# kopacja/rho2sdf.jl

Measured on AMD Instinct MI355X. Metric: Mvoxels/s SDF extract on 512^3 grid over 100k HEX8; max|err| vs ref, higher is better.
Workload: dtype f64

## Files before the change

rho2sdf.jl_amd/csrc/rho2sdf_hip.hip:

```cpp
#include <hip/hip_runtime.h>

#include <algorithm>
#include <cmath>
#include <cstdarg>
#include <cstddef>
#include <cstdio>
#include <cstring>
#include <initializer_list>
#include <utility>
#include <string>
#include <vector>

#include "../../include/rho2sdf_hip.h"
#include "r2s_common.hpp"
#include "r2s_device_math.hpp"

#include <type_traits>

using namespace r2s;

__constant__ int c_hex_isn[6][4] = {{0, 3, 2, 1}, {0, 1, 5, 4}, {1, 2, 6, 5},
                                    {2, 3, 7, 6}, {3, 0, 4, 7}, {4, 5, 6, 7}};

#define SCAN_BLOCK 256
// ... 1305 lines not shown
            for (int k = 0; k < 8; ++k) t = fma(E.X[k][q], N[k], t);
            xp[q] = t;
        }
        res[slot] = norm3(x[0] - xp[0], x[1] - xp[1], x[2] - xp[2]);
        if (res_xp) {
            res_xp[3 * slot] = xp[0];
            res_xp[3 * slot + 1] = xp[1];
            res_xp[3 * slot + 2] = xp[2];
        }
    }
}

struct alignas(16) SignBox {
    int32_t lo[3];
    int32_t dim[3];
    double rmax;
};

__device__ __forceinline__ bool coord_range(const GridDev& g, int ax, double mn, double mx, int nmax, int& a, int& b)
{
    const double fa = ceil((mn - g.amin[ax]) / g.cell), fb = floor((mx - g.amin[ax]) / g.cell);
    if (!(fa <= (double)nmax + 2.0) || !(fb >= -2.0)) return false;
    a = (fa < 0.0) ? 0 : ((fa > (double)nmax) ? nmax : (int)fa);
    b = (fb > (double)nmax) ? nmax : ((fb < 0.0) ? 0 : (int)fb);
    while (a > 0 && grid_coord(g, ax, a - 1) >= mn) --a;
    while (a <= nmax && grid_coord(g, ax, a) < mn) ++a;
    while (b < nmax && grid_coord(g, ax, b + 1) <= mx) ++b;
    while (b >= 0 && grid_coord(g, ax, b) > mx) --b;
    return a <= b;
}

__global__ void sign_box_kernel(const ElemRec* __restrict__ erec, uint32_t nel, GridDev g, SlabInfo s,
                                const uint8_t* __restrict__ hot, SignBox* __restrict__ sbox,
                                uint32_t* __restrict__ nchunks, uint32_t* __restrict__ nstore)
{
    const uint32_t gid = blockIdx.x * blockDim.x + threadIdx.x;
    const uint32_t el = gid / BIN_LANES, sub = gid % BIN_LANES;
    const bool live = el < nel;
    SignBox B;
    memset(&B, 0, sizeof B);
    const ElemRec& E = erec[live ? el : 0];
    int lo[3], hi[3];
    bool found = false;
    if (live && sign_tile_range(E, g, s, lo, hi)) {
        const uint32_t n = tile_count(lo, hi);
        for (uint32_t q = sub; q < n && !found; q += BIN_LANES) found = hot[tile_of(lo, hi, q, s)] != 0;
    }
    const unsigned long long m = __ballot(found);
    const bool rel = ((m >> ((threadIdx.x & 63u) & ~(unsigned)(BIN_LANES - 1))) & ((1ull << BIN_LANES) - 1ull)) != 0;
    if (!live || sub != 0) return;
    if (rel) {
        const int nmax[3] = {g.nx - 1, g.ny - 1, g.nz - 1};
        uint64_t vol = 1;
        for (int ax = 0; ax < 3; ++ax) {
            int a = 0, b = -1;
            if (coord_range(g, ax, E.mn[ax], E.mx[ax], nmax[ax], a, b)) {
                if (ax == 2) {
                    int la, lb;
                    if (slab_local_range(s, a, b, la, lb)) { a = la; b = lb; }
                    else { a = 0; b = -1; }
                }
            } else { a = 0; b = -1; }
            B.lo[ax] = a;
            B.dim[ax] = (b >= a) ? (b - a + 1) : 0;
            vol *= (uint64_t)B.dim[ax];
        }
        if (vol == 0) B.dim[0] = B.dim[1] = B.dim[2] = 0;
        nchunks[el] = (uint32_t)((vol + 63) / 64);
        const TileBox tb = tile_box(B.lo, B.dim);
        nstore[el] = vol ? (uint32_t)(tb.td[0] * tb.td[1] * tb.td[2]) : 0u;
    }
    B.rmax = E.rmax;
    sbox[el] = B;
}

__global__ void __launch_bounds__(64) sign_project_kernel(const SignBox* __restrict__ sbox, uint32_t nel,
                                                          const uint32_t* __restrict__ chunk_off, uint32_t nchunks,
                                                          const uint32_t* __restrict__ store_off,
                                                          uint32_t cpw, const ElemRec* __restrict__ erec, GridDev g,
                                                          SlabInfo sl, double rho_t, const uint8_t* __restrict__ hot,
                                                          double* __restrict__ res, const uint32_t* __restrict__ abort_flag)
{
    const uint32_t ab = *abort_flag;
    __shared__ uint32_t queue[128];
    const uint32_t w = __builtin_amdgcn_readfirstlane((blockIdx.x * blockDim.x + threadIdx.x) >> 6);
    uint32_t c = w * cpw;
    if (c >= nchunks) return;
    const uint32_t c_end = (c + cpw < nchunks) ? c + cpw : nchunks;
    uint32_t lo = 0, hi = nel;
    while (hi - lo > 1) {
        const uint32_t mid = (lo + hi) >> 1;
        if (chunk_off[mid] <= c) lo = mid; else hi = mid;
    }
    if (ab) return;
    const uint32_t lane = threadIdx.x & 63;
    while (c < c_end) {
        lo = __builtin_amdgcn_readfirstlane(lo);
        const SignBox& B = sbox[lo];
        const ElemRec& E = erec[lo];
        const uint32_t co = chunk_off[lo], cn = chunk_off[lo + 1];
        const uint32_t seg_end = (cn < c_end) ? cn : c_end;
        const BoxDecode dec = box_decode_make((uint32_t)B.dim[0], (uint32_t)B.dim[1], (uint32_t)B.dim[2]);
        const uint32_t vol = dec.bxy * (uint32_t)B.dim[2];
        const uint32_t v_begin = (c - co) * 64u;
        const uint32_t v_end = ((seg_end - co) * 64u < vol) ? (seg_end - co) * 64u : vol;
        const int lo0 = B.lo[0], lo1 = B.lo[1], lo2 = B.lo[2];
        const uint32_t st_off = store_off[lo];
        const TileBox tb = tile_box(B.lo, B.dim);
        const double margin = 1e-9 * fmax(1.0, fabs(rho_t));
        const double uniform_sign = (E.rmin > rho_t + margin) ? 1.0 : ((E.rmax < rho_t - margin) ? -1.0 : 0.0);
        uint32_t qn = 0;
        for (uint32_t v0 = v_begin; v0 < v_end || qn > 0; v0 += 64u) {
            if (v0 < v_end) {
                const uint32_t v = v0 + lane;
                bool pass = false;
                if (v < v_end) {
                    uint32_t li, lj, lk;
                    box_decode(dec, v, li, lj, lk);
                    const int i = lo0 + (int)li, j = lo1 + (int)lj, kl = lo2 + (int)lk;
                    double x[3];
                    x[0] = grid_coord(g, 0, i);
                    x[1] = grid_coord(g, 1, j);
                    x[2] = grid_coord(g, 2, slab_global_k(sl, kl));
                    const uint32_t t = ((uint32_t)(kl >> 2) * sl.nty + (uint32_t)(j >> 2)) * sl.ntx + (uint32_t)(i >> 2);
                    pass = hot[t] && !hex8_outside(E, x);
                    if (!pass) res[tile_slot(st_off, tb, i, j, kl)] = INFINITY;
                    else if (uniform_sign != 0.0 && hex8_inner(E, x)) {
                        res[tile_slot(st_off, tb, i, j, kl)] = uniform_sign > 0.0 ? 0.0 : -0.0;
                        pass = false;
                    }
                }
                const uint64_t m = __ballot(pass);
                if (pass) queue[qn + __builtin_amdgcn_mbcnt_hi((uint32_t)(m >> 32), __builtin_amdgcn_mbcnt_lo((uint32_t)m, 0u))] = v;
                qn += (uint32_t)__popcll(m);
                __syncthreads();
            }
            if (qn >= 64u || (v0 + 64u >= v_end && qn > 0)) {
                const uint32_t take = qn < 64u ? qn : 64u;
                const bool have = lane < take;
                const uint32_t v = queue[lane];
                const uint32_t spill = queue[64u + lane];
                __syncthreads();
                if (lane + 64u < qn) queue[lane] = spill;
                qn -= take;
                __syncthreads();
                if (have) {
                    uint32_t li, lj, lk;
                    box_decode(dec, v, li, lj, lk);
                    const int i = lo0 + (int)li, j = lo1 + (int)lj, kl = lo2 + (int)lk;
                    double x[3], xi[3], N[8];
                    x[0] = grid_coord(g, 0, i);
                    x[1] = grid_coord(g, 1, j);
                    x[2] = grid_coord(g, 2, slab_global_k(sl, kl));
                    inv_map_hex8(E, x, xi);
                    const double m = fmax(fabs(xi[0]), fmax(fabs(xi[1]), fabs(xi[2])));
                    double val = INFINITY;
                    if (m < 1.01) {
                        hex8_shape(xi, N);
                        double rho = 0.0;
#pragma unroll
                        for (int k = 0; k < 8; ++k) rho += N[k] * E.r[k];
                        val = (rho >= rho_t) ? m : -m;
                    }
                    res[tile_slot(st_off, tb, i, j, kl)] = val;
                }
            }
        }
        c = seg_end;
        if (c < c_end) {
            do { ++lo; } while (chunk_off[lo + 1] <= c);
        }
    }
}

#define AT_ITEMS 8
__global__ void __launch_bounds__(256) active_tiles_kernel(const uint32_t* __restrict__ band_cnt,
                                                           const uint32_t* __restrict__ sign_cnt,
                                                           const uint8_t* __restrict__ hot, uint32_t ntiles,
                                                           uint32_t* __restrict__ active_band,
                                                           uint32_t* __restrict__ active_sign,
                                                           uint32_t* __restrict__ active_any,
                                                           uint32_t* __restrict__ active_sonly,
                                                           const uint8_t* __restrict__ tri,
                                                           uint32_t* __restrict__ active_lean,
                                                           uint32_t* __restrict__ active_tri,
                                                           uint32_t* __restrict__ counters)
{
    __shared__ uint32_t s_cnt[6][AT_ITEMS][4], s_base[6], s_max[2];
    if (threadIdx.x < 2) s_max[threadIdx.x] = 0;
    const int lane = threadIdx.x & 63, wave = threadIdx.x >> 6;
    const unsigned long long below = (1ull << lane) - 1ull;
    const uint32_t t0 = blockIdx.x * (256u * AT_ITEMS);
    uint32_t mxb = 0, mxs = 0;
    uint32_t flags[AT_ITEMS];
#pragma unroll
    for (int i = 0; i < AT_ITEMS; ++i) {
        const uint32_t t = t0 + (uint32_t)i * 256u + threadIdx.x;
        const bool in = t < ntiles;
        const uint32_t bc = in ? band_cnt[t] : 0u, sc = in ? sign_cnt[t] : 0u;
        const bool f[3] = {bc != 0, sc != 0 && hot[t] != 0, false};
        const bool ft = f[0] && tri[t] != 0;
        const bool fl[6] = {f[0], f[1], f[0] || f[1], f[1] && !f[0], f[0] && !ft, ft};
        uint32_t fb = 0;
// ... 388 lines not shown
    const uint32_t* __restrict__ ids = reinterpret_cast<const uint32_t*>(seg + 2 + (int64_t)cap_full * 64);
    const int lane = threadIdx.x & 63;
    const int ntx = (nx + 3) / 4, nty = (ny + 3) / 4;
    const uint32_t t = ids[w];
    const int tx = t % ntx, ty = (t / ntx) % nty, tz = t / (ntx * nty);
    const int i = tx * 4 + (lane & 3), j = ty * 4 + ((lane >> 2) & 3), k = tz * 4 + (lane >> 4);
    if (i < nx && j < ny && k < nz) volume[((int64_t)k * ny + j) * nx + i] = payload[(size_t)w * 64 + lane];
}
__global__ void __launch_bounds__(256) unpack_segments_masks_kernel(const double* __restrict__ buf, int64_t seglen, uint32_t cap_full,
                                                                   uint32_t cap_mask, int nx, int ny, int nz, double magnitude,
                                                                   double* __restrict__ volume)
{
    const double* __restrict__ seg = buf + (int64_t)blockIdx.y * seglen;
    const int64_t nf = reinterpret_cast<const int64_t*>(seg)[0], nm = reinterpret_cast<const int64_t*>(seg)[1];
    const uint32_t w = __builtin_amdgcn_readfirstlane((blockIdx.x * blockDim.x + threadIdx.x) >> 6);
    if (nf < 0 || nf > (int64_t)cap_full || nm < 0 || nm > (int64_t)cap_mask || (int64_t)w >= nm) return;
    const uint64_t* __restrict__ masks = reinterpret_cast<const uint64_t*>(seg + 2 + (int64_t)cap_full * 64 + (cap_full + 1) / 2);
    const uint32_t* __restrict__ ids = reinterpret_cast<const uint32_t*>(masks + cap_mask);
    const int lane = threadIdx.x & 63;
    const int ntx = (nx + 3) / 4, nty = (ny + 3) / 4;
    const uint32_t t = ids[w];
    const int tx = t % ntx, ty = (t / ntx) % nty, tz = t / (ntx * nty);
    const int i = tx * 4 + (lane & 3), j = ty * 4 + ((lane >> 2) & 3), k = tz * 4 + (lane >> 4);
    if (i < nx && j < ny && k < nz) volume[((int64_t)k * ny + j) * nx + i] = ((masks[w] >> lane) & 1ull) ? magnitude : -magnitude;
}

struct r2s_plan {
    int device = 0;
    int n_cu = 256;
    DevBuf deg, ine_ptr, ine, cursor, erec, cls, fmask, nitems, item_off, items;
    DevBuf band_cnt, band_off, band_raw, band_ent, sign_cnt, sign_off, sign_raw, sign_ent;
    DevBuf active, active_sign, active_any, active_sonly, active_lean, active_tri, tri, hot, counters, scan_tmp[3], scan_tmp2[3], nchunks, chunk_off, iso_res, iso_res_xp, strag;
    DevBuf perm, wchunks, hardflag;
    DevBuf sbox, s_nchunks, s_chunk_off, sres;
    DevBuf nstore, store_off, s_nstore, s_store_off;
    SlabInfo last_s;
    GridDev last_g;
    uint32_t last_n_any = 0, last_n_band = 0, last_n_sonly = 0;
    bool has_last = false;
    uint32_t* h_pinned = nullptr;
    uint32_t* d_pinned = nullptr;
    struct Spec {
        bool valid = false;
        int64_t key[12] = {0};
        uint32_t v[16] = {0};
    } spec;
    hipEvent_t ev[8] = {nullptr, nullptr, nullptr, nullptr, nullptr, nullptr, nullptr, nullptr};
    hipStream_t st2 = nullptr;
    hipStream_t st3 = nullptr;
    hipEvent_t ev2[8] = {nullptr, nullptr, nullptr, nullptr, nullptr, nullptr, nullptr, nullptr};
    hipEvent_t ev_fast[2] = {nullptr, nullptr};
    bool fast_timed = false;
};

static int scan_exclusive2(r2s_plan* P, const uint32_t* in0, uint32_t* out0, const uint32_t* in1, uint32_t* out1,
                           int64_t n, hipStream_t st, int level = 0, int bank = 0)
{
    DevBuf* tmp = bank ? P->scan_tmp2 : P->scan_tmp;
    if (n <= 0) return 0;
    const unsigned ny = in1 ? 2u : 1u;
    const int64_t nb = (n + SCAN_TILE - 1) / SCAN_TILE;
    ScanPair sp;
    sp.in[0] = in0; sp.out[0] = out0; sp.in[1] = in1; sp.out[1] = out1;
    sp.sums[0] = sp.sums[1] = nullptr;
    if (nb == 1) {
        scan_block_kernel<<<dim3(1, ny), SCAN_BLOCK, 0, st>>>(sp, n);
        return 0;
// ... 108 lines not shown
    int rc = check_device(device);
    if (rc) return rc;
    HIP_TRY(hipSetDevice(device));
    r2s_plan* P = new r2s_plan();
    P->device = device;
    {
        hipDeviceProp_t prop;
        if (hipGetDeviceProperties(&prop, device) == hipSuccess && prop.multiProcessorCount > 0) P->n_cu = prop.multiProcessorCount;
    }
    HIP_TRY(hipHostMalloc((void**)&P->h_pinned, 128, hipHostMallocMapped | hipHostMallocCoherent));
    HIP_TRY(hipHostGetDevicePointer((void**)&P->d_pinned, P->h_pinned, 0));
    for (int i = 0; i < 8; ++i) HIP_TRY(hipEventCreate(&P->ev[i]));
    for (int i = 0; i < 8; ++i) HIP_TRY(hipEventCreate(&P->ev2[i]));
    for (int i = 0; i < 2; ++i) HIP_TRY(hipEventCreate(&P->ev_fast[i]));
    {
        int prio_lo = 0, prio_hi = 0;
        HIP_TRY(hipDeviceGetStreamPriorityRange(&prio_lo, &prio_hi));
        (void)prio_lo;
        HIP_TRY(hipStreamCreateWithPriority(&P->st2, hipStreamNonBlocking, prio_hi));
        HIP_TRY(hipStreamCreateWithFlags(&P->st3, hipStreamNonBlocking));
    }
    *out = P;
    return 0;
}

void r2s_plan_destroy(r2s_plan* P)
{
    if (!P) return;
    (void)hipSetDevice(P->device);
    DevBuf* all[] = {&P->deg, &P->ine_ptr, &P->ine, &P->cursor, &P->erec, &P->cls, &P->fmask, &P->nitems,
                     &P->item_off, &P->items, &P->band_cnt, &P->band_off, &P->band_raw, &P->band_ent,
                     &P->sign_cnt, &P->sign_off, &P->sign_raw, &P->sign_ent, &P->active, &P->active_sign, &P->active_any, &P->active_sonly, &P->active_lean, &P->active_tri, &P->tri,
                     &P->hot, &P->counters, &P->nchunks, &P->chunk_off, &P->iso_res, &P->iso_res_xp, &P->strag,
                     &P->perm, &P->wchunks, &P->hardflag, &P->sbox, &P->s_nchunks, &P->s_chunk_off, &P->sres, &P->nstore, &P->store_off, &P->s_nstore, &P->s_store_off,
                     &P->scan_tmp[0], &P->scan_tmp[1], &P->scan_tmp[2], &P->scan_tmp2[0], &P->scan_tmp2[1], &P->scan_tmp2[2]};
    for (DevBuf* b : all) b->release();
    if (P->h_pinned) (void)hipHostFree(P->h_pinned);
    for (int i = 0; i < 8; ++i)
        if (P->ev[i]) (void)hipEventDestroy(P->ev[i]);
    for (int i = 0; i < 8; ++i)
        if (P->ev2[i]) (void)hipEventDestroy(P->ev2[i]);
    for (int i = 0; i < 2; ++i)
        if (P->ev_fast[i]) (void)hipEventDestroy(P->ev_fast[i]);
    if (P->st2) (void)hipStreamDestroy(P->st2);
    if (P->st3) (void)hipStreamDestroy(P->st3);
    delete P;
}


}

static uint32_t iso_straggler_cap(uint32_t n_store)
{
    static const int cap_env = getenv("R2S_ISO_STRAGGLER_CAP") ? atoi(getenv("R2S_ISO_STRAGGLER_CAP")) : 0;
    if (cap_env > 0) return (uint32_t)cap_env;
    const uint64_t slots = 64ull * std::max<uint32_t>(n_store, 1u);
    return (uint32_t)std::max<uint64_t>(slots / 16, std::min<uint64_t>(slots, 1ull << 20));
}

static int iso_project_hex(r2s_plan* P, hipStream_t st, uint32_t n_items, uint32_t n_chunks, uint32_t n_store, uint32_t wps,
                           const GridDev& g, const SlabInfo& s, double rho_t, double* res_xp, uint32_t* counters,
                           const uint32_t* abort_flag)
{
    static const int free_env = getenv("R2S_ISO_FREE") ? atoi(getenv("R2S_ISO_FREE")) : 0;
    const uint32_t resident = (uint32_t)P->n_cu * 4u * wps - (uint32_t)std::min(std::max(free_env, 0), (int)P->n_cu * 4);
    static const int group_env = getenv("R2S_ISO_GROUP") ? atoi(getenv("R2S_ISO_GROUP")) : 0;
    const uint32_t group = group_env > 0 ? (uint32_t)group_env
// ... 125 lines not shown
    elem_prep_kernel<ET><<<(unsigned)((nel + 127) / 128), 128, 0, st>>>(
        dX, dIEN, d_rho_n, nel, nnp, rho_t, g, P->erec.as<typename ET::Rec>(),
        P->cls.as<uint8_t>(), P->fmask.as<uint32_t>(), P->nitems.as<uint32_t>(), s, delta);
    HIP_TRY(hipEventRecord(P->ev2[5], st));
    HIP_TRY(hipStreamWaitEvent(P->st2, P->ev2[0], 0));
    {
        const int64_t n = nel * ET::NEN;
        node_degree_kernel<<<(unsigned)((n + 255) / 256), 256, 0, P->st2>>>(dIEN, nel, ET::NEN, nnp, P->deg.as<uint32_t>(), (int*)counters);
        int rc = scan_exclusive(P, P->deg.as<uint32_t>(), P->ine_ptr.as<uint32_t>(), nnp + 1, P->st2);
        if (rc) return rc;
        ine_fill_kernel<<<(unsigned)((n + 255) / 256), 256, 0, P->st2>>>(dIEN, nel, ET::NEN, nnp, P->ine_ptr.as<uint32_t>(), P->cursor.as<uint32_t>(), P->ine.as<uint32_t>());
    }
    HIP_TRY(hipEventRecord(P->ev2[1], P->st2));
    if constexpr (std::is_same<typename ET::Rec, ElemRec>::value) {
        HIP_TRY(hipStreamWaitEvent(P->st2, P->ev2[5], 0));
        HIP_TRY(hipStreamWaitEvent(P->st3, P->ev2[5], 0));
        static const int no_inner_env = getenv("R2S_SIGN_NO_INNER") ? atoi(getenv("R2S_SIGN_NO_INNER")) : 0;
        hex_planes_kernel<<<(unsigned)((nel * 6 + 255) / 256), 256, 0, P->st3>>>(P->erec.as<ElemRec>(), nel,
                                                                                 (no_inner_env || prm.sign_no_inner) ? 1 : 0);
        HIP_TRY(hipEventRecord(P->ev2[5], P->st3));
    }
    constexpr bool HEX = std::is_same<typename ET::Rec, ElemRec>::value;
    const double rmax_needed = HEX ? -INFINITY : rho_t - 1e-12 * (fabs(rho_t) + 1.0);
    const bool sign_items = HEX && want_sign && nel > 0;
    ReadBack rb2;
    if constexpr (HEX) {
        if (sign_items) {
            zero_many(P->st2, {{P->sign_cnt.p, sizeof(uint32_t) * (size_t)(ntiles + 1)}, {P->hot.p, (size_t)ntiles + 1}});
            sign_hot_kernel<ElemRec><<<(unsigned)((nel * BIN_LANES + 255) / 256), 256, 0, P->st2>>>(P->erec.as<ElemRec>(), (uint32_t)nel, g, s, rho_t, P->hot.as<uint8_t>());
            sign_bin_kernel<ElemRec, false><<<(unsigned)((nel * BIN_LANES + 255) / 256), 256, 0, P->st2>>>(P->erec.as<ElemRec>(), (uint32_t)nel, g, s, P->sign_cnt.as<uint32_t>(), nullptr, nullptr, P->hot.as<uint8_t>(), abort_flag, rmax_needed);
            int rc = scan_exclusive2(P, P->sign_cnt.as<uint32_t>(), P->sign_off.as<uint32_t>(), nullptr, nullptr, (int64_t)ntiles + 1, P->st2, 0, 1);
            if (rc) return rc;
            ENSURE(P->sbox, sizeof(SignBox) * (size_t)nel);
            ENSURE(P->s_nchunks, sizeof(uint32_t) * (size_t)(nel + 1));
            ENSURE(P->s_chunk_off, sizeof(uint32_t) * (size_t)(nel + 1));
            ENSURE(P->s_nstore, sizeof(uint32_t) * (size_t)(nel + 1));
            ENSURE(P->s_store_off, sizeof(uint32_t) * (size_t)(nel + 1));
            zero_many(P->st2, {{P->s_nchunks.p, sizeof(uint32_t) * (size_t)(nel + 1)}, {P->s_nstore.p, sizeof(uint32_t) * (size_t)(nel + 1)}});
            sign_box_kernel<<<(unsigned)((nel * BIN_LANES + 255) / 256), 256, 0, P->st2>>>(P->erec.as<ElemRec>(), (uint32_t)nel, g, s, P->hot.as<uint8_t>(), P->sbox.as<SignBox>(), P->s_nchunks.as<uint32_t>(), P->s_nstore.as<uint32_t>());
            rc = scan_exclusive2(P, P->s_nchunks.as<uint32_t>(), P->s_chunk_off.as<uint32_t>(), P->s_nstore.as<uint32_t>(),
                                 P->s_store_off.as<uint32_t>(), nel + 1, P->st2, 0, 1);
            if (rc) return rc;
            rb2.add(P->s_chunk_off.as<uint32_t>() + nel, 1, 11);
            rb2.add(P->s_store_off.as<uint32_t>() + nel, 1, 13);
            HIP_TRY(hipEventRecord(P->ev2[7], P->st2));
        }
    }
    HIP_TRY(hipStreamWaitEvent(st, P->ev2[1], 0));
    face_mask_kernel<ET><<<(unsigned)((nel * ET::NES + 255) / 256), 256, 0, st>>>(
        dIEN, nel, P->ine_ptr.as<uint32_t>(), P->ine.as<uint32_t>(), P->cls.as<uint8_t>(), P->fmask.as<uint32_t>(),
        P->nitems.as<uint32_t>(), (const int*)counters);
    {
        int rc = scan_exclusive(P, P->nitems.as<uint32_t>(), P->item_off.as<uint32_t>(), nel + 1, st);
        if (rc) return rc;
    }
    {
        ReadBack rb;
        rb.add(P->item_off.as<uint32_t>() + nel, 1, 0);
        rb.add(counters, 1, 1);
        read_back_kernel<<<1, 64, 0, st>>>(rb, P->d_pinned, ex, counters + 15);
    }
    if (!spec) {
        HIP_TRY(hipStreamSynchronize(st));
        if (P->h_pinned[1]) return fail(R2S_ERR_ARG, "IEN contains node ids outside 1..nnp");
        cnt[0] = P->h_pinned[0];
        cnt[1] = 0;
    }
    const uint32_t n_items = want_dist ? cnt[0] : 0;
    ENSURE(P->items, sizeof(BandItem) * (size_t)std::max<uint32_t>(n_items, 1));
    ENSURE(P->nchunks, sizeof(uint32_t) * (size_t)(n_items + 1));
    ENSURE(P->chunk_off, sizeof(uint32_t) * (size_t)(n_items + 1));
    ENSURE(P->nstore, sizeof(uint32_t) * (size_t)(n_items + 1));
    ENSURE(P->store_off, sizeof(uint32_t) * (size_t)(n_items + 1));
    if (n_items) {
        ENSURE(P->hardflag, (size_t)n_items + 1);
        zero_many(st, {{P->nchunks.p, sizeof(uint32_t) * (size_t)(n_items + 1)}, {P->nstore.p, sizeof(uint32_t) * (size_t)(n_items + 1)},
                       {P->hardflag.p, (size_t)n_items + 1}});
        item_build_kernel<ET><<<(unsigned)((nel + 63) / 64), 64, 0, st>>>(
            P->erec.as<typename ET::Rec>(), P->cls.as<uint8_t>(), P->fmask.as<uint32_t>(), P->item_off.as<uint32_t>(), nel,
            g, s, delta, P->items.as<BandItem>(), P->nchunks.as<uint32_t>(), P->nstore.as<uint32_t>(), P->hardflag.as<uint8_t>(), rho_t, abort_flag);
        const uint32_t* work_counts = P->nchunks.as<uint32_t>();
        if constexpr (std::is_same<typename ET::Rec, ElemRec>::value) {
            ENSURE(P->perm, sizeof(uint32_t) * (size_t)n_items);
            ENSURE(P->wchunks, sizeof(uint32_t) * (size_t)(n_items + 1));
            work_order_kernel<<<1, 1024, 0, st>>>(P->hardflag.as<uint8_t>(), P->nchunks.as<uint32_t>(), n_items,
                                                  P->perm.as<uint32_t>(), P->wchunks.as<uint32_t>());
            work_counts = P->wchunks.as<uint32_t>();
        }
        int rc = scan_exclusive2(P, work_counts, P->chunk_off.as<uint32_t>(), P->nstore.as<uint32_t>(),
                                 P->store_off.as<uint32_t>(), (int64_t)n_items + 1, st);
        if (rc) return rc;
        item_chunks_kernel<<<(n_items + 255) / 256, 256, 0, st>>>(P->items.as<BandItem>(), P->chunk_off.as<uint32_t>(), P->store_off.as<uint32_t>(), n_items);
        rb2.add(P->chunk_off.as<uint32_t>() + n_items, 1, 10);
        rb2.add(P->store_off.as<uint32_t>() + n_items, 1, 12);
    }
    HIP_TRY(hipEventRecord(P->ev[1], st));

    static const bool overlap_env0 = !(getenv("R2S_NO_OVERLAP") && atoi(getenv("R2S_NO_OVERLAP")));
    static const bool early_env = !(getenv("R2S_NO_EARLY_ISO") && atoi(getenv("R2S_NO_EARLY_ISO")));
    bool early_iso = false;
    if constexpr (std::is_same<typename ET::Rec, ElemRec>::value) {
        early_iso = spec && early_env && overlap_env0 && want_sign && want_dist && nel > 0 && n_items && cnt[10] && cnt[11] && !(mode & R2S_OUT_XP);
        if (early_iso) {
            ReadBack rbA;
            rbA.add(P->chunk_off.as<uint32_t>() + n_items, 1, 10);
            rbA.add(P->store_off.as<uint32_t>() + n_items, 1, 12);
            read_back_kernel<<<1, 64, 0, st>>>(rbA, P->d_pinned, ex, counters + 15);
            HIP_TRY(hipEventRecord(P->ev2[6], st));
            const uint32_t n_chunks_e = cnt[10], n_store_e = cnt[12];
            ENSURE(P->iso_res, sizeof(double) * 64 * (size_t)std::max<uint32_t>(n_store_e, 1));
            static const int wps_env = getenv("R2S_ISO_WPS") ? atoi(getenv("R2S_ISO_WPS")) : 0;
            const uint32_t wps = (wps_env >= 1 && wps_env <= 3) ? (uint32_t)wps_env : 2u;
            if (sign_items) HIP_TRY(hipStreamWaitEvent(st, P->ev2[7], 0));
            HIP_TRY(hipEventRecord(P->ev[7], st));
            { const int rc = iso_project_hex(P, st, n_items, n_chunks_e, n_store_e, wps, g, s, rho_t, nullptr, counters, abort_flag); if (rc) return rc; }
            HIP_TRY(hipEventRecord(P->ev[6], st));
            HIP_TRY(hipStreamWaitEvent(P->st2, P->ev2[6], 0));
        }
    } else {
        early_iso = spec && early_env && overlap_env0 && mode == R2S_OUT_SDF && want_sign && want_dist && n_items && cnt[10];
        if (early_iso) {
            ReadBack rbA;
            rbA.add(P->chunk_off.as<uint32_t>() + n_items, 1, 10);
            rbA.add(P->store_off.as<uint32_t>() + n_items, 1, 12);
            read_back_kernel<<<1, 64, 0, st>>>(rbA, P->d_pinned, ex, counters + 15);
            HIP_TRY(hipEventRecord(P->ev2[6], st));
            const uint32_t n_chunks_e = cnt[10], n_store_e = cnt[12];
            ENSURE(P->iso_res, sizeof(double) * 64 * (size_t)std::max<uint32_t>(n_store_e, 1));
            static const int cpw_env = getenv("R2S_ISO_CPW") ? atoi(getenv("R2S_ISO_CPW")) : 0;
            const uint32_t cpw = cpw_env > 0 ? (uint32_t)cpw_env : 8u;
            const uint32_t nwaves = (n_chunks_e + cpw - 1) / cpw;
            HIP_TRY(hipEventRecord(P->ev[7], st));
            iso_project_kernel<typename ET::Rec><<<(nwaves + 3) / 4, 256, 0, st>>>(
                P->items.as<BandItem>(), n_items, P->chunk_off.as<uint32_t>(), n_chunks_e, P->erec.as<typename ET::Rec>(), g,
                s, rho_t, P->iso_res.as<double>(), nullptr, abort_flag, cpw);
// ... 9 lines not shown
            band_bin_kernel<false><<<(n_items * BIN_LANES + 127) / 128, 128, 0, bs>>>(P->items.as<BandItem>(), n_items, g, s, P->band_cnt.as<uint32_t>(), nullptr, nullptr, P->tri.as<uint8_t>(), abort_flag);
        int rc = scan_exclusive2(P, P->band_cnt.as<uint32_t>(), P->band_off.as<uint32_t>(), nullptr, nullptr, (int64_t)ntiles + 1, bs);
        if (rc) return rc;
        HIP_TRY(hipStreamWaitEvent(bs, P->ev2[7], 0));
    } else {
        zero_many(bs, {{P->band_cnt.p, sizeof(uint32_t) * (size_t)(ntiles + 1)}, {P->sign_cnt.p, sizeof(uint32_t) * (size_t)(ntiles + 1)},
                       {P->hot.p, (size_t)ntiles + 1}, {P->tri.p, (size_t)ntiles + 1}});
        if (n_items)
            band_bin_kernel<false><<<(n_items * BIN_LANES + 127) / 128, 128, 0, bs>>>(P->items.as<BandItem>(), n_items, g, s, P->band_cnt.as<uint32_t>(), nullptr, nullptr, P->tri.as<uint8_t>(), abort_flag);
        if (want_sign)
        {
            sign_hot_kernel<typename ET::Rec><<<(unsigned)((nel * BIN_LANES + 255) / 256), 256, 0, bs>>>(P->erec.as<typename ET::Rec>(), (uint32_t)nel, g, s, rho_t, P->hot.as<uint8_t>());
            sign_bin_kernel<typename ET::Rec, false><<<(unsigned)((nel * BIN_LANES + 255) / 256), 256, 0, bs>>>(P->erec.as<typename ET::Rec>(), (uint32_t)nel, g, s, P->sign_cnt.as<uint32_t>(), nullptr, nullptr, P->hot.as<uint8_t>(), abort_flag, rmax_needed);
        }
        int rc = scan_exclusive2(P, P->band_cnt.as<uint32_t>(), P->band_off.as<uint32_t>(), P->sign_cnt.as<uint32_t>(),
                                 P->sign_off.as<uint32_t>(), (int64_t)ntiles + 1, bs);
        if (rc) return rc;
    }
    active_tiles_kernel<<<(ntiles + 256 * AT_ITEMS - 1) / (256 * AT_ITEMS), 256, 0, bs>>>(P->band_cnt.as<uint32_t>(), P->sign_cnt.as<uint32_t>(), P->hot.as<uint8_t>(), ntiles, P->active.as<uint32_t>(), P->active_sign.as<uint32_t>(), P->active_any.as<uint32_t>(), P->active_sonly.as<uint32_t>(), P->tri.as<uint8_t>(), P->active_lean.as<uint32_t>(), P->active_tri.as<uint32_t>(), counters);
    rb2.add(P->band_off.as<uint32_t>() + ntiles, 1, 2);
    rb2.add(P->sign_off.as<uint32_t>() + ntiles, 1, 3);
    rb2.add(counters + 1, 6, 4);
    rb2.add(counters + 10, 2, 14);
    read_back_kernel<<<1, 64, 0, bs>>>(rb2, P->d_pinned, ex, counters + 15);
    if (!spec) {
        HIP_TRY(hipStreamSynchronize(bs));
        for (int q = 2; q < 16; ++q) cnt[q] = P->h_pinned[q];
    }
    const uint32_t n_band = cnt[2], n_sign = cnt[3], n_active = cnt[4], n_active_sign = cnt[5];
    P->last_s = s; P->last_g = g; P->last_n_any = cnt[8]; P->last_n_band = cnt[4]; P->last_n_sonly = cnt[9]; P->has_last = true;
    const uint32_t n_chunks = n_items ? cnt[10] : 0;
    const uint32_t n_store = n_items ? cnt[12] : 0;
    ENSURE(P->iso_res, sizeof(double) * 64 * (size_t)std::max<uint32_t>(n_store, 1));
    const uint32_t n_schunks = sign_items ? cnt[11] : 0;
    const uint32_t n_sstore = sign_items ? cnt[13] : 0;
    if (sign_items) ENSURE(P->sres, sizeof(double) * 64 * (size_t)std::max<uint32_t>(n_sstore, 1));
    if (mode & R2S_OUT_XP) ENSURE(P->iso_res_xp, sizeof(double) * 192 * (size_t)std::max<uint32_t>(n_store, 1));
    ENSURE(P->band_raw, sizeof(uint32_t) * (size_t)std::max<uint32_t>(n_band, 1));
    ENSURE(P->band_ent, sizeof(uint32_t) * (size_t)std::max<uint32_t>(n_band, 1));
    ENSURE(P->sign_raw, sizeof(uint32_t) * (size_t)std::max<uint32_t>(n_sign, 1));
    ENSURE(P->sign_ent, sizeof(uint32_t) * (size_t)std::max<uint32_t>(n_sign, 1));
    zero_many(bs, {{P->band_cnt.p, sizeof(uint32_t) * (size_t)(ntiles + 1)}, {P->sign_cnt.p, sizeof(uint32_t) * (size_t)(ntiles + 1)}});
    if (n_items)
        band_bin_kernel<true><<<(n_items * BIN_LANES + 127) / 128, 128, 0, bs>>>(P->items.as<BandItem>(), n_items, g, s, P->band_cnt.as<uint32_t>(), P->band_off.as<uint32_t>(), P->band_raw.as<uint32_t>(), nullptr, abort_flag);
    if (want_sign)
        sign_bin_kernel<typename ET::Rec, true><<<(unsigned)((nel * BIN_LANES + 255) / 256), 256, 0, bs>>>(P->erec.as<typename ET::Rec>(), (uint32_t)nel, g, s, P->sign_cnt.as<uint32_t>(), P->sign_off.as<uint32_t>(), HEX ? P->sign_raw.as<uint32_t>() : P->sign_ent.as<uint32_t>(), P->hot.as<uint8_t>(), abort_flag, rmax_needed);
    if (n_active) {
        bin_sort_small_kernel<<<(n_active * SORT_LANES + 255) / 256, 256, 0, bs>>>(P->active.as<uint32_t>(), n_active, P->band_off.as<uint32_t>(), P->band_raw.as<uint32_t>(), P->band_ent.as<uint32_t>(), abort_flag);
        if (cnt[6] > 64u)
            bin_sort_kernel<<<(n_active + 3) / 4, 256, 0, bs>>>(P->active.as<uint32_t>(), n_active, P->band_off.as<uint32_t>(), P->band_raw.as<uint32_t>(), P->band_ent.as<uint32_t>(), abort_flag);
    }
    if (n_active_sign && HEX) {
        bin_sort_small_kernel<<<(n_active_sign * SORT_LANES + 255) / 256, 256, 0, bs>>>(P->active_sign.as<uint32_t>(), n_active_sign, P->sign_off.as<uint32_t>(), P->sign_raw.as<uint32_t>(), P->sign_ent.as<uint32_t>(), abort_flag);
        if (cnt[7] > 64u)
            bin_sort_kernel<<<(n_active_sign + 3) / 4, 256, 0, bs>>>(P->active_sign.as<uint32_t>(), n_active_sign, P->sign_off.as<uint32_t>(), P->sign_raw.as<uint32_t>(), P->sign_ent.as<uint32_t>(), abort_flag);
    }
    HIP_TRY(hipEventRecord(P->ev[2], bs));

    static const bool overlap_env = !(getenv("R2S_NO_OVERLAP") && atoi(getenv("R2S_NO_OVERLAP")));
    const bool overlap = !HEX && overlap_env && mode == R2S_OUT_SDF && want_sign && want_dist;
    const bool fork = HEX && overlap_env && want_sign && want_dist && n_chunks && n_schunks;
    {
        const bool two_streams = overlap || fork;
        hipStream_t fs = two_streams ? P->st2 : st;
        const unsigned fill_grid = 256 * 8;
        if (two_streams) HIP_TRY(hipStreamWaitEvent(P->st2, P->ev[2], 0));
        HIP_TRY(hipEventRecord(P->ev2[0], fs));
        if (mode & R2S_OUT_DIST) fill_kernel<<<fill_grid, 256, 0, fs>>>(d_dist, nvox, 1.0e10);
        if (mode & R2S_OUT_SIGN) fill_kernel<<<fill_grid, 256, 0, fs>>>(d_sign, nvox, -1.0);
        if (mode & R2S_OUT_SDF) fill_kernel<<<fill_grid, 256, 0, fs>>>(d_sdf, nvox, -1.0e10);
        if (mode & R2S_OUT_XP) HIP_TRY(hipMemsetAsync(d_xp, 0, sizeof(double) * 3 * (size_t)nvox, fs));
        HIP_TRY(hipEventRecord(P->ev2[3], fs));
        HIP_TRY(hipEventRecord(P->ev[3], st));
        if (two_streams) HIP_TRY(hipEventRecord(P->ev2[1], P->st2));
    }

    {
        MainArgs A;
        A.g = g; A.s = s; A.rho_t = rho_t;
        A.true_min = prm.true_min ? 1 : 0;
        A.band_off = P->band_off.as<uint32_t>(); A.band_ent = P->band_ent.as<uint32_t>();
        A.sign_off = P->sign_off.as<uint32_t>(); A.sign_ent = P->sign_ent.as<uint32_t>();
        A.items = P->items.as<BandItem>(); A.erec = P->erec.as<typename ET::Rec>();
        A.dist = (mode & R2S_OUT_DIST) ? d_dist : nullptr;
        A.sign = (mode & R2S_OUT_SIGN) ? d_sign : nullptr;
        A.sdf = (mode & R2S_OUT_SDF) ? d_sdf : nullptr;
        A.sbox = P->sbox.p; A.s_store_off = P->s_store_off.as<uint32_t>(); A.sres = P->sres.as<double>();
        A.hot = P->hot.as<uint8_t>();
        A.abort_flag = abort_flag;
        if constexpr (HEX) {
            hipStream_t ss = fork ? P->st2 : st;
            if (!fork) HIP_TRY(hipEventRecord(P->ev2[1], ss));
            if (want_sign && n_schunks) {
                const uint32_t cpw = 8, nwaves = (n_schunks + cpw - 1) / cpw;
                HIP_TRY(hipStreamWaitEvent(ss, P->ev2[5], 0));
                sign_project_kernel<<<nwaves, 64, 0, ss>>>(P->sbox.as<SignBox>(), (uint32_t)nel, P->s_chunk_off.as<uint32_t>(), n_schunks, P->s_store_off.as<uint32_t>(), cpw,
                                                          P->erec.as<ElemRec>(), g, s, rho_t, P->hot.as<uint8_t>(), P->sres.as<double>(), abort_flag);
            }
            HIP_TRY(hipEventRecord(P->ev2[4], ss));
            A.xp = (mode & R2S_OUT_XP) ? d_xp : nullptr;
            A.sdf_mode = 1;
            const uint32_t n_sonly = cnt[9];
            const bool early_sign_tiles = want_dist && want_sign && !(mode & R2S_OUT_XP);
            if (early_sign_tiles && n_sonly) {
                MainArgs B = A;
                B.active = P->active_sonly.as<uint32_t>(); B.n_active = n_sonly;
                sdf_tiles_kernel<ElemRec, false, true><<<n_sonly, 64, 0, ss>>>(B);
            }
            HIP_TRY(hipEventRecord(P->ev2[2], ss));
            A.iso_res = P->iso_res.as<double>();
            A.iso_res_xp = (mode & R2S_OUT_XP) ? P->iso_res_xp.as<double>() : nullptr;
            if (!early_iso) HIP_TRY(hipEventRecord(P->ev[7], st));
            if (want_dist && n_chunks && !early_iso) {
                static const int wps_env = getenv("R2S_ISO_WPS") ? atoi(getenv("R2S_ISO_WPS")) : 0;
                const uint32_t wps = (wps_env >= 1 && wps_env <= 3) ? (uint32_t)wps_env : 3u;
                if (fork) HIP_TRY(hipStreamWaitEvent(st, P->ev2[0], 0));
                double* const res_xp = (mode & R2S_OUT_XP) ? P->iso_res_xp.as<double>() : nullptr;
                { const int rc = iso_project_hex(P, st, n_items, n_chunks, n_store, wps, g, s, rho_t, res_xp, counters, abort_flag); if (rc) return rc; }
            }
            if (!early_iso) HIP_TRY(hipEventRecord(P->ev[6], st));
            if (fork) HIP_TRY(hipStreamWaitEvent(st, P->ev2[4], 0));
            if (want_dist && want_sign && early_sign_tiles) {
                const uint32_t n_lean = cnt[14], n_tri = cnt[15];
                if (n_lean) {
                    A.active = P->active_lean.as<uint32_t>(); A.n_active = n_lean;
                    sdf_tiles_kernel<ElemRec, true, true, false><<<n_lean, 64, 0, st>>>(A);
                }
                if (n_tri) {
                    A.active = P->active_tri.as<uint32_t>(); A.n_active = n_tri;
                    if (A.true_min) sdf_tiles_kernel<ElemRec, true, true, true, true><<<(n_tri + 3) / 4, 256, 0, st>>>(A);
// ... 236 lines not shown
```

Before: 33660.

## Restructure sign projection to iterate 4x4x4 tiles with per-tile plane culling

The sign projection kernel now distributes work over 4x4x4 storage tiles instead of linear 64-voxel chunks. For each tile it does a conservative face-plane test to classify the whole tile as outside, fully inner, or mixed, and writes outside or inner tiles without per-voxel tests. Mixed tiles are processed lane-per-voxel, with Newton candidates queued in a wave-local LDS ring buffer synchronized by s_waitcnt instead of __syncthreads. Chunk-count buffers and their scan are removed, and the default tiles per wave rises from 8 to 16. The tile-level test adds work for tiles that end up mixed, and the classification has to match the per-voxel results.

```diff
diff --git a/rho2sdf.jl_amd/csrc/rho2sdf_hip.hip b/rho2sdf.jl_amd/csrc/rho2sdf_hip.hip
--- a/rho2sdf.jl_amd/csrc/rho2sdf_hip.hip
+++ b/rho2sdf.jl_amd/csrc/rho2sdf_hip.hip
@@ -1361,7 +1361,7 @@
 
 __global__ void sign_box_kernel(const ElemRec* __restrict__ erec, uint32_t nel, GridDev g, SlabInfo s,
                                 const uint8_t* __restrict__ hot, SignBox* __restrict__ sbox,
-                                uint32_t* __restrict__ nchunks, uint32_t* __restrict__ nstore)
+                                uint32_t* __restrict__ ntile)
 {
     const uint32_t gid = blockIdx.x * blockDim.x + threadIdx.x;
     const uint32_t el = gid / BIN_LANES, sub = gid % BIN_LANES;
@@ -1395,109 +1395,163 @@
             vol *= (uint64_t)B.dim[ax];
         }
         if (vol == 0) B.dim[0] = B.dim[1] = B.dim[2] = 0;
-        nchunks[el] = (uint32_t)((vol + 63) / 64);
         const TileBox tb = tile_box(B.lo, B.dim);
-        nstore[el] = vol ? (uint32_t)(tb.td[0] * tb.td[1] * tb.td[2]) : 0u;
+        ntile[el] = vol ? (uint32_t)(tb.td[0] * tb.td[1] * tb.td[2]) : 0u;
     }
     B.rmax = E.rmax;
     sbox[el] = B;
 }
 
+__device__ __forceinline__ void wave_lds_sync() { asm volatile("s_waitcnt lgkmcnt(0)" ::: "memory"); }
+
+struct SignQueue {
+    uint4 e[128];
+};
+
+__device__ __forceinline__ void sign_newton_batch(const ElemRec& E, const GridDev& g, const SlabInfo& sl, double rho_t,
+                                                  SignQueue& Q, uint32_t& qh, uint32_t& qn, uint32_t lane,
+                                                  double* __restrict__ line0)
+{
+    const uint32_t take = qn < 64u ? qn : 64u;
+    const uint4 e = Q.e[(qh + lane) & 127u];
+    wave_lds_sync();
+    const bool have = lane < take;
+    qh = (qh + take) & 127u;
+    qn -= take;
+    if (have) {
+        const int i = (int)e.y, j = (int)e.z, kl = (int)e.w;
+        double x[3], xi[3], N[8];
+        x[0] = grid_coord(g, 0, i);
+        x[1] = grid_coord(g, 1, j);
+        x[2] = grid_coord(g, 2, slab_global_k(sl, kl));
+        inv_map_hex8(E, x, xi);
+        const double m = fmax(fabs(xi[0]), fmax(fabs(xi[1]), fabs(xi[2])));
+        double val = INFINITY;
+        if (m < 1.01) {
+            hex8_shape(xi, N);
+            double rho = 0.0;
+#pragma unroll
+            for (int k = 0; k < 8; ++k) rho += N[k] * E.r[k];
+            val = (rho >= rho_t) ? m : -m;
+        }
+        line0[(size_t)e.x * 64u + (uint32_t)((i & 3) | ((j & 3) << 2) | ((kl & 3) << 4))] = val;
+    }
+}
+
 __global__ void __launch_bounds__(64) sign_project_kernel(const SignBox* __restrict__ sbox, uint32_t nel,
-                                                          const uint32_t* __restrict__ chunk_off, uint32_t nchunks,
-                                                          const uint32_t* __restrict__ store_off,
+                                                          const uint32_t* __restrict__ tile_off, uint32_t ntiles_all,
                                                           uint32_t cpw, const ElemRec* __restrict__ erec, GridDev g,
                                                           SlabInfo sl, double rho_t, const uint8_t* __restrict__ hot,
-                                                          double* __restrict__ res, const uint32_t* __restrict__ abort_flag)
+                                                          int dense_store, double* __restrict__ res,
+                                                          const uint32_t* __restrict__ abort_flag)
 {
     const uint32_t ab = *abort_flag;
-    __shared__ uint32_t queue[128];
+    __shared__ SignQueue Q;
     const uint32_t w = __builtin_amdgcn_readfirstlane((blockIdx.x * blockDim.x + threadIdx.x) >> 6);
     uint32_t c = w * cpw;
-    if (c >= nchunks) return;
-    const uint32_t c_end = (c + cpw < nchunks) ? c + cpw : nchunks;
+    if (c >= ntiles_all) return;
+    const uint32_t c_end = (c + cpw < ntiles_all) ? c + cpw : ntiles_all;
     uint32_t lo = 0, hi = nel;
     while (hi - lo > 1) {
         const uint32_t mid = (lo + hi) >> 1;
-        if (chunk_off[mid] <= c) lo = mid; else hi = mid;
+        if (tile_off[mid] <= c) lo = mid; else hi = mid;
     }
     if (ab) return;
     const uint32_t lane = threadIdx.x & 63;
+    const int lx = (int)(lane & 3u), ly = (int)((lane >> 2) & 3u), lz = (int)(lane >> 4);
+    uint32_t qh = 0, qn = 0;
     while (c < c_end) {
         lo = __builtin_amdgcn_readfirstlane(lo);
         const SignBox& B = sbox[lo];
         const ElemRec& E = erec[lo];
-        const uint32_t co = chunk_off[lo], cn = chunk_off[lo + 1];
+        const uint32_t co = tile_off[lo], cn = tile_off[lo + 1];
         const uint32_t seg_end = (cn < c_end) ? cn : c_end;
-        const BoxDecode dec = box_decode_make((uint32_t)B.dim[0], (uint32_t)B.dim[1], (uint32_t)B.dim[2]);
-        const uint32_t vol = dec.bxy * (uint32_t)B.dim[2];
-        const uint32_t v_begin = (c - co) * 64u;
-        const uint32_t v_end = ((seg_end - co) * 64u < vol) ? (seg_end - co) * 64u : vol;
         const int lo0 = B.lo[0], lo1 = B.lo[1], lo2 = B.lo[2];
-        const uint32_t st_off = store_off[lo];
+        const uint32_t d0 = (uint32_t)B.dim[0], d1 = (uint32_t)B.dim[1], d2 = (uint32_t)B.dim[2];
         const TileBox tb = tile_box(B.lo, B.dim);
+        const BoxDecode dec = box_decode_make((uint32_t)tb.td[0], (uint32_t)tb.td[1], (uint32_t)tb.td[2]);
+        double* __restrict__ const line0 = res + (size_t)co * 64u;
         const double margin = 1e-9 * fmax(1.0, fabs(rho_t));
         const double uniform_sign = (E.rmin > rho_t + margin) ? 1.0 : ((E.rmax < rho_t - margin) ? -1.0 : 0.0);
-        uint32_t qn = 0;
-        for (uint32_t v0 = v_begin; v0 < v_end || qn > 0; v0 += 64u) {
-            if (v0 < v_end) {
-                const uint32_t v = v0 + lane;
+        const double inner_val = uniform_sign > 0.0 ? 0.0 : -0.0;
+        const uint32_t q_end = seg_end - co;
+        for (uint32_t q0 = c - co; q0 < q_end; q0 += 64u) {
+            uint32_t code = 0;
+            int tx = 0, ty = 0, tz = 0;
+            if (q0 + lane < q_end) {
+                uint32_t ta, tb1, tc;
+                box_decode(dec, q0 + lane, ta, tb1, tc);
+                tx = tb.t0[0] + (int)ta; ty = tb.t0[1] + (int)tb1; tz = tb.t0[2] + (int)tc;
+                const uint32_t t = ((uint32_t)tz * sl.nty + (uint32_t)ty) * sl.ntx + (uint32_t)tx;
+                if (hot[t] && !tile_clear_of(E, g, sl, tx, ty, tz)) {
+                    const int a0[3] = {max(4 * tx, lo0), max(4 * ty, lo1), max(4 * tz, lo2)};
+                    const int a1[3] = {min(4 * tx + 3, lo0 + (int)d0 - 1), min(4 * ty + 3, lo1 + (int)d1 - 1),
+                                       min(4 * tz + 3, lo2 + (int)d2 - 1)};
+                    const double xa[3] = {grid_coord(g, 0, a0[0]), grid_coord(g, 1, a0[1]), grid_coord(g, 2, slab_global_k(sl, a0[2]))};
+                    const double xb[3] = {grid_coord(g, 0, a1[0]), grid_coord(g, 1, a1[1]), grid_coord(g, 2, slab_global_k(sl, a1[2]))};
+                    bool all_out = false, all_in = true;
+#pragma unroll
+                    for (int f = 0; f < 6; ++f) {
+                        double xmax[3], xmin[3];
+#pragma unroll
+                        for (int q = 0; q < 3; ++q) {
+                            const bool neg = E.pn[f][q] < 0.0;
+                            xmax[q] = neg ? xa[q] : xb[q];
+                            xmin[q] = neg ? xb[q] : xa[q];
+                        }
+                        const double vmax = E.pn[f][0] * xmax[0] + E.pn[f][1] * xmax[1] + E.pn[f][2] * xmax[2];
+                        const double vmin = E.pn[f][0] * xmin[0] + E.pn[f][1] * xmin[1] + E.pn[f][2] * xmin[2];
+                        all_out = all_out || (vmin > E.po[f]);
+                        all_in = all_in && (vmax <= E.pi[f]) && !(vmax > E.po[f]);
+                    }
+                    code = all_out ? 1u : ((all_in && uniform_sign != 0.0) ? 2u : 3u);
+                } else if (dense_store) {
+                    code = 1u;
+                }
+            }
+            for (uint64_t m_work = __ballot(code != 0u); m_work; m_work &= m_work - 1ull) {
+                const int tl = (int)__builtin_ctzll(m_work);
+                const uint32_t cd = (uint32_t)__builtin_amdgcn_readlane((int)code, tl);
+                const int i = 4 * __builtin_amdgcn_readlane(tx, tl) + lx, j = 4 * __builtin_amdgcn_readlane(ty, tl) + ly,
+                          kl = 4 * __builtin_amdgcn_readlane(tz, tl) + lz;
+                const bool inb = (uint32_t)(i - lo0) < d0 && (uint32_t)(j - lo1) < d1 && (uint32_t)(kl - lo2) < d2;
+                const uint32_t q = q0 + (uint32_t)tl;
+                double* __restrict__ const slot = line0 + (size_t)q * 64u + lane;
+                if (cd != 3u) {
+                    if (inb) *slot = (cd == 1u) ? (double)INFINITY : inner_val;
+                    continue;
+                }
                 bool pass = false;
-                if (v < v_end) {
-                    uint32_t li, lj, lk;
-                    box_decode(dec, v, li, lj, lk);
-                    const int i = lo0 + (int)li, j = lo1 + (int)lj, kl = lo2 + (int)lk;
+                if (inb) {
                     double x[3];
                     x[0] = grid_coord(g, 0, i);
                     x[1] = grid_coord(g, 1, j);
                     x[2] = grid_coord(g, 2, slab_global_k(sl, kl));
-                    const uint32_t t = ((uint32_t)(kl >> 2) * sl.nty + (uint32_t)(j >> 2)) * sl.ntx + (uint32_t)(i >> 2);
-                    pass = hot[t] && !hex8_outside(E, x);
-                    if (!pass) res[tile_slot(st_off, tb, i, j, kl)] = INFINITY;
+                    pass = !hex8_outside(E, x);
+                    if (!pass) *slot = INFINITY;
                     else if (uniform_sign != 0.0 && hex8_inner(E, x)) {
-                        res[tile_slot(st_off, tb, i, j, kl)] = uniform_sign > 0.0 ? 0.0 : -0.0;
+                        *slot = inner_val;
                         pass = false;
                     }
                 }
+#ifdef R2S_SIGN_SCAN_ONLY
+                pass = false;
+#endif
                 const uint64_t m = __ballot(pass);
-                if (pass) queue[qn + __builtin_amdgcn_mbcnt_hi((uint32_t)(m >> 32), __builtin_amdgcn_mbcnt_lo((uint32_t)m, 0u))] = v;
-                qn += (uint32_t)__popcll(m);
-                __syncthreads();
-            }
-            if (qn >= 64u || (v0 + 64u >= v_end && qn > 0)) {
-                const uint32_t take = qn < 64u ? qn : 64u;
-                const bool have = lane < take;
-                const uint32_t v = queue[lane];
-                const uint32_t spill = queue[64u + lane];
-                __syncthreads();
-                if (lane + 64u < qn) queue[lane] = spill;
-                qn -= take;
-                __syncthreads();
-                if (have) {
-                    uint32_t li, lj, lk;
-                    box_decode(dec, v, li, lj, lk);
-                    const int i = lo0 + (int)li, j = lo1 + (int)lj, kl = lo2 + (int)lk;
-                    double x[3], xi[3], N[8];
-                    x[0] = grid_coord(g, 0, i);
-                    x[1] = grid_coord(g, 1, j);
-                    x[2] = grid_coord(g, 2, slab_global_k(sl, kl));
-                    inv_map_hex8(E, x, xi);
-                    const double m = fmax(fabs(xi[0]), fmax(fabs(xi[1]), fabs(xi[2])));
-                    double val = INFINITY;
-                    if (m < 1.01) {
-                        hex8_shape(xi, N);
-                        double rho = 0.0;
-#pragma unroll
-                        for (int k = 0; k < 8; ++k) rho += N[k] * E.r[k];
-                        val = (rho >= rho_t) ? m : -m;
-                    }
-                    res[tile_slot(st_off, tb, i, j, kl)] = val;
+                if (m) {
+                    if (pass)
+                        Q.e[(qh + qn + __builtin_amdgcn_mbcnt_hi((uint32_t)(m >> 32), __builtin_amdgcn_mbcnt_lo((uint32_t)m, 0u))) & 127u] =
+                            make_uint4(q, (uint32_t)i, (uint32_t)j, (uint32_t)kl);
+                    qn += (uint32_t)__popcll(m);
+                    wave_lds_sync();
+                    if (qn >= 64u) sign_newton_batch(E, g, sl, rho_t, Q, qh, qn, lane, line0);
                 }
             }
         }
+        if (qn > 0) sign_newton_batch(E, g, sl, rho_t, Q, qh, qn, lane, line0);
         c = seg_end;
         if (c < c_end) {
-            do { ++lo; } while (chunk_off[lo + 1] <= c);
+            do { ++lo; } while (tile_off[lo + 1] <= c);
         }
     }
 }
@@ -1952,7 +2006,7 @@
     DevBuf band_cnt, band_off, band_raw, band_ent, sign_cnt, sign_off, sign_raw, sign_ent;
     DevBuf active, active_sign, active_any, active_sonly, active_lean, active_tri, tri, hot, counters, scan_tmp[3], scan_tmp2[3], nchunks, chunk_off, iso_res, iso_res_xp, strag;
     DevBuf perm, wchunks, hardflag;
-    DevBuf sbox, s_nchunks, s_chunk_off, sres;
+    DevBuf sbox, sres;
     DevBuf nstore, store_off, s_nstore, s_store_off;
     SlabInfo last_s;
     GridDev last_g;
@@ -2127,7 +2181,7 @@
                      &P->item_off, &P->items, &P->band_cnt, &P->band_off, &P->band_raw, &P->band_ent,
                      &P->sign_cnt, &P->sign_off, &P->sign_raw, &P->sign_ent, &P->active, &P->active_sign, &P->active_any, &P->active_sonly, &P->active_lean, &P->active_tri, &P->tri,
                      &P->hot, &P->counters, &P->nchunks, &P->chunk_off, &P->iso_res, &P->iso_res_xp, &P->strag,
-                     &P->perm, &P->wchunks, &P->hardflag, &P->sbox, &P->s_nchunks, &P->s_chunk_off, &P->sres, &P->nstore, &P->store_off, &P->s_nstore, &P->s_store_off,
+                     &P->perm, &P->wchunks, &P->hardflag, &P->sbox, &P->sres, &P->nstore, &P->store_off, &P->s_nstore, &P->s_store_off,
                      &P->scan_tmp[0], &P->scan_tmp[1], &P->scan_tmp[2], &P->scan_tmp2[0], &P->scan_tmp2[1], &P->scan_tmp2[2]};
     for (DevBuf* b : all) b->release();
     if (P->h_pinned) (void)hipHostFree(P->h_pinned);
@@ -2319,16 +2373,12 @@
             int rc = scan_exclusive2(P, P->sign_cnt.as<uint32_t>(), P->sign_off.as<uint32_t>(), nullptr, nullptr, (int64_t)ntiles + 1, P->st2, 0, 1);
             if (rc) return rc;
             ENSURE(P->sbox, sizeof(SignBox) * (size_t)nel);
-            ENSURE(P->s_nchunks, sizeof(uint32_t) * (size_t)(nel + 1));
-            ENSURE(P->s_chunk_off, sizeof(uint32_t) * (size_t)(nel + 1));
             ENSURE(P->s_nstore, sizeof(uint32_t) * (size_t)(nel + 1));
             ENSURE(P->s_store_off, sizeof(uint32_t) * (size_t)(nel + 1));
-            zero_many(P->st2, {{P->s_nchunks.p, sizeof(uint32_t) * (size_t)(nel + 1)}, {P->s_nstore.p, sizeof(uint32_t) * (size_t)(nel + 1)}});
-            sign_box_kernel<<<(unsigned)((nel * BIN_LANES + 255) / 256), 256, 0, P->st2>>>(P->erec.as<ElemRec>(), (uint32_t)nel, g, s, P->hot.as<uint8_t>(), P->sbox.as<SignBox>(), P->s_nchunks.as<uint32_t>(), P->s_nstore.as<uint32_t>());
-            rc = scan_exclusive2(P, P->s_nchunks.as<uint32_t>(), P->s_chunk_off.as<uint32_t>(), P->s_nstore.as<uint32_t>(),
-                                 P->s_store_off.as<uint32_t>(), nel + 1, P->st2, 0, 1);
+            zero_many(P->st2, {{P->s_nstore.p, sizeof(uint32_t) * (size_t)(nel + 1)}});
+            sign_box_kernel<<<(unsigned)((nel * BIN_LANES + 255) / 256), 256, 0, P->st2>>>(P->erec.as<ElemRec>(), (uint32_t)nel, g, s, P->hot.as<uint8_t>(), P->sbox.as<SignBox>(), P->s_nstore.as<uint32_t>());
+            rc = scan_exclusive2(P, P->s_nstore.as<uint32_t>(), P->s_store_off.as<uint32_t>(), nullptr, nullptr, nel + 1, P->st2, 0, 1);
             if (rc) return rc;
-            rb2.add(P->s_chunk_off.as<uint32_t>() + nel, 1, 11);
             rb2.add(P->s_store_off.as<uint32_t>() + nel, 1, 13);
             HIP_TRY(hipEventRecord(P->ev2[7], P->st2));
         }
@@ -2387,7 +2437,7 @@
     static const bool early_env = !(getenv("R2S_NO_EARLY_ISO") && atoi(getenv("R2S_NO_EARLY_ISO")));
     bool early_iso = false;
     if constexpr (std::is_same<typename ET::Rec, ElemRec>::value) {
-        early_iso = spec && early_env && overlap_env0 && want_sign && want_dist && nel > 0 && n_items && cnt[10] && cnt[11] && !(mode & R2S_OUT_XP);
+        early_iso = spec && early_env && overlap_env0 && want_sign && want_dist && nel > 0 && n_items && cnt[10] && cnt[13] && !(mode & R2S_OUT_XP);
         if (early_iso) {
             ReadBack rbA;
             rbA.add(P->chunk_off.as<uint32_t>() + n_items, 1, 10);
@@ -2463,7 +2513,6 @@
     const uint32_t n_chunks = n_items ? cnt[10] : 0;
     const uint32_t n_store = n_items ? cnt[12] : 0;
     ENSURE(P->iso_res, sizeof(double) * 64 * (size_t)std::max<uint32_t>(n_store, 1));
-    const uint32_t n_schunks = sign_items ? cnt[11] : 0;
     const uint32_t n_sstore = sign_items ? cnt[13] : 0;
     if (sign_items) ENSURE(P->sres, sizeof(double) * 64 * (size_t)std::max<uint32_t>(n_sstore, 1));
     if (mode & R2S_OUT_XP) ENSURE(P->iso_res_xp, sizeof(double) * 192 * (size_t)std::max<uint32_t>(n_store, 1));
@@ -2490,7 +2539,7 @@
 
     static const bool overlap_env = !(getenv("R2S_NO_OVERLAP") && atoi(getenv("R2S_NO_OVERLAP")));
     const bool overlap = !HEX && overlap_env && mode == R2S_OUT_SDF && want_sign && want_dist;
-    const bool fork = HEX && overlap_env && want_sign && want_dist && n_chunks && n_schunks;
+    const bool fork = HEX && overlap_env && want_sign && want_dist && n_chunks && n_sstore;
     {
         const bool two_streams = overlap || fork;
         hipStream_t fs = two_streams ? P->st2 : st;
@@ -2522,11 +2571,14 @@
         if constexpr (HEX) {
             hipStream_t ss = fork ? P->st2 : st;
             if (!fork) HIP_TRY(hipEventRecord(P->ev2[1], ss));
-            if (want_sign && n_schunks) {
-                const uint32_t cpw = 8, nwaves = (n_schunks + cpw - 1) / cpw;
+            if (want_sign && n_sstore) {
+                static const int cpw_env = getenv("R2S_SIGN_CPW") ? atoi(getenv("R2S_SIGN_CPW")) : 0;
+                const char* dense_s = getenv("R2S_SIGN_DENSE_STORE");
+                const int dense_env = dense_s ? atoi(dense_s) : 0;
+                const uint32_t cpw = cpw_env > 0 ? (uint32_t)cpw_env : 16u, nwaves = (n_sstore + cpw - 1) / cpw;
                 HIP_TRY(hipStreamWaitEvent(ss, P->ev2[5], 0));
-                sign_project_kernel<<<nwaves, 64, 0, ss>>>(P->sbox.as<SignBox>(), (uint32_t)nel, P->s_chunk_off.as<uint32_t>(), n_schunks, P->s_store_off.as<uint32_t>(), cpw,
-                                                          P->erec.as<ElemRec>(), g, s, rho_t, P->hot.as<uint8_t>(), P->sres.as<double>(), abort_flag);
+                sign_project_kernel<<<nwaves, 64, 0, ss>>>(P->sbox.as<SignBox>(), (uint32_t)nel, P->s_store_off.as<uint32_t>(), n_sstore, cpw,
+                                                          P->erec.as<ElemRec>(), g, s, rho_t, P->hot.as<uint8_t>(), dense_env ? 1 : 0, P->sres.as<double>(), abort_flag);
             }
             HIP_TRY(hipEventRecord(P->ev2[4], ss));
             A.xp = (mode & R2S_OUT_XP) ? d_xp : nullptr;
```

After: 31100. -7.6%, worse.
